# JeffreyXiang/ivid

Hardware: NVIDIA H100
Metric: 128x128 RGBD multiview samples/sec (higher is better)
Workload: dtype fp16 tensor-core operands, fp32 accumulate / residual stream / GroupNorm / softmax / sampler

## Files before the change

ivid_b200/csrc/elementwise.cuh:

```cuda
#pragma once
#include "common.cuh"

namespace ivid {

constexpr int kStatsPixPerBlock = 256;

__global__ void __launch_bounds__(256) gn_stats_kernel(const float* __restrict__ x, double* __restrict__ stats,
                                                       int HW, int C) {
  __shared__ float sred[256 * 8];
  const int n = blockIdx.y;
  const int c4 = C >> 2;
  const int cols = c4 < 256 ? c4 : 256;
  const int rows = 256 / cols;
  const int tx = threadIdx.x % cols;
  const int ty = threadIdx.x / cols;
  const int p0 = blockIdx.x * kStatsPixPerBlock;
  const int p1 = min(p0 + kStatsPixPerBlock, HW);
  const float* base = x + (static_cast<size_t>(n) * HW) * C;
  for (int cc = tx; cc < c4; cc += cols) {
    float s[4] = {0.f, 0.f, 0.f, 0.f}, q[4] = {0.f, 0.f, 0.f, 0.f};
    if (ty < rows) {
      for (int p = p0 + ty; p < p1; p += rows) {
        const float4 v = ldg_f4(base + static_cast<size_t>(p) * C + cc * 4);
        s[0] += v.x; s[1] += v.y; s[2] += v.z; s[3] += v.w;
        q[0] += v.x * v.x; q[1] += v.y * v.y; q[2] += v.z * v.z; q[3] += v.w * v.w;
      }
    }
    float* sm = sred;
    if (ty < rows) {
#pragma unroll
      for (int j = 0; j < 4; ++j) {
        sm[(ty * cols + tx) * 8 + j] = s[j];
        sm[(ty * cols + tx) * 8 + 4 + j] = q[j];
      }
    }
    __syncthreads();
    if (ty == 0) {
      double ds[4], dq[4];
#pragma unroll
      for (int j = 0; j < 4; ++j) { ds[j] = 0.0; dq[j] = 0.0; }
      for (int r = 0; r < rows; ++r) {
#pragma unroll
        for (int j = 0; j < 4; ++j) {
          ds[j] += static_cast<double>(sm[(r * cols + tx) * 8 + j]);
          dq[j] += static_cast<double>(sm[(r * cols + tx) * 8 + 4 + j]);
        }
      }
      double* o = stats + (static_cast<size_t>(n) * C + cc * 4) * 2;
#pragma unroll
      for (int j = 0; j < 4; ++j) {
        atomicAdd(o + 2 * j, ds[j]);
        atomicAdd(o + 2 * j + 1, dq[j]);
      }
    }
    __syncthreads();
  }
}

struct GnApplyParams {
  const float* x0; const float* x1;
  const __half* x0h; const __half* x1h;
  int C0, C1;
  int N, H, W;
  int mode;
  int silu;
  const double* stats0; const double* stats1;
  int groups; double inv_count; float eps;
  const float* gamma; const float* beta;
  const float* film; int film_ld, film_off;
  int film_add;
  int pix_per_block;
  __half* out_act;
  __half* out_lo;
  __half* out_raw16;
  float* out_raw32;
  uint8_t* out_act8;
};

template <bool kF8> struct Act8 { using T = uint4; };
template <> struct Act8<true> { using T = uint2; };
template <bool kF8>
__device__ __forceinline__ typename Act8<kF8>::T pack_act8(const float (&a)[8]) {
  if constexpr (kF8) {
    uint2 pk;
    pk.x = pack_e4m3x2(a[0], a[1]) | (static_cast<uint32_t>(pack_e4m3x2(a[2], a[3])) << 16);
    pk.y = pack_e4m3x2(a[4], a[5]) | (static_cast<uint32_t>(pack_e4m3x2(a[6], a[7])) << 16);
    return pk;
  } else {
    uint4 pk;
    pk.x = pack_h2(a[0], a[1]); pk.y = pack_h2(a[2], a[3]);
    pk.z = pack_h2(a[4], a[5]); pk.w = pack_h2(a[6], a[7]);
    return pk;
  }
}
template <bool kF8>
__device__ __forceinline__ void store_act8(const GnApplyParams& p, size_t o, const typename Act8<kF8>::T& v) {
  if constexpr (kF8) *reinterpret_cast<uint2*>(p.out_act8 + o) = v;
  else *reinterpret_cast<uint4*>(p.out_act + o) = v;
}

__device__ __forceinline__ void load8(const GnApplyParams& p, int n, int h, int w, int c, float (&v)[8]) {
  if (p.x0h != nullptr) {
    const __half* hs; int hc, hl;
    if (c < p.C0) { hs = p.x0h; hc = c; hl = p.C0; } else { hs = p.x1h; hc = c - p.C0; hl = p.C1; }
    const uint4 u = __ldg(reinterpret_cast<const uint4*>(hs + ((static_cast<size_t>(n) * p.H + h) * p.W + w) * hl + hc));
    const __half2* h2 = reinterpret_cast<const __half2*>(&u);
#pragma unroll
    for (int j = 0; j < 4; ++j) { const float2 f = __half22float2(h2[j]); v[2 * j] = f.x; v[2 * j + 1] = f.y; }
    return;
  }
  const float* src;
  int cc, ld;
  if (c < p.C0) { src = p.x0; cc = c; ld = p.C0; } else { src = p.x1; cc = c - p.C0; ld = p.C1; }
  const float* q = src + ((static_cast<size_t>(n) * p.H + h) * p.W + w) * ld + cc;
  const float4 a = ldg_f4(q), b = ldg_f4(q + 4);
  v[0] = a.x; v[1] = a.y; v[2] = a.z; v[3] = a.w; v[4] = b.x; v[5] = b.y; v[6] = b.z; v[7] = b.w;
}

__device__ __forceinline__ void gn_block_pos(const GnApplyParams&, int& n, int& bx) {
  n = static_cast<int>(blockIdx.y);
  bx = static_cast<int>(blockIdx.x);
}

__device__ __forceinline__ void gn_prologue(const GnApplyParams& p, float* s_ab, float* s_mean, float* s_rstd) {
  const int C = p.C0 + p.C1;
  int n, bx_unused;
  gn_block_pos(p, n, bx_unused);
  const int cpg = C / p.groups;
  if ((cpg & (cpg - 1)) == 0 && cpg <= 32 && C % 32 == 0 && C <= 4 * 256 && blockDim.x == 256) {
    constexpr int PF = 4;
    double2 st[PF];
    float pg[PF], pb[PF], psc[PF], psh[PF];
#pragma unroll
    for (int i = 0; i < PF; ++i) {
      const int c = threadIdx.x + i * 256;
      if (c < C) {
        const double* sp = (c < p.C0) ? p.stats0 + (static_cast<size_t>(n) * p.C0 + c) * 2
                                      : p.stats1 + (static_cast<size_t>(n) * p.C1 + (c - p.C0)) * 2;
        st[i] = *reinterpret_cast<const double2*>(sp);
        pg[i] = p.gamma[c];
        pb[i] = p.beta[c];
        if (p.film != nullptr) {
          psc[i] = p.film[static_cast<size_t>(n) * p.film_ld + p.film_off + c];
          psh[i] = p.film_add ? 0.f : p.film[static_cast<size_t>(n) * p.film_ld + p.film_off + C + c];
          if (p.film_add) {
            const double e = static_cast<double>(psc[i]), hw = 1.0 / p.inv_count;
            const double S = st[i].x;
            st[i].x = S + hw * e;
            st[i].y = st[i].y + 2.0 * e * S + hw * e * e;
          }
        }
      }
    }
    const double cnt_inv = p.inv_count / cpg;
#pragma unroll
    for (int i = 0; i < PF; ++i) {
      const int c = threadIdx.x + i * 256;
      if (c < C) {
        double sm = st[i].x, q = st[i].y;
        for (int off = 1; off < cpg; off <<= 1) {
          sm += __shfl_xor_sync(0xffffffffu, sm, off);
          q += __shfl_xor_sync(0xffffffffu, q, off);
        }
        const double mean = sm * cnt_inv;
        double var = q * cnt_inv - mean * mean;
        if (var < 0.0) var = 0.0;
        const float rstd = static_cast<float>(1.0 / sqrt(var + static_cast<double>(p.eps)));
        const float a0 = rstd * pg[i];
        const float b0 = pb[i] - static_cast<float>(mean) * a0;
        float av = a0, bv = b0;
        if (p.film != nullptr && p.film_add) {
          bv = fmaf(psc[i], a0, b0);
        } else if (p.film != nullptr) {
          const float sc = 1.0f + psc[i];
          av = a0 * sc;
          bv = b0 * sc + psh[i];
        }
        s_ab[(c & 7) * (C >> 3) + (c >> 3)] = av;
        s_ab[C + (c & 7) * (C >> 3) + (c >> 3)] = bv;
      }
    }
    __syncthreads();
    return;
  }
  for (int g = threadIdx.x; g < p.groups; g += blockDim.x) {
    double s = 0.0, q = 0.0;
    for (int c = g * cpg; c < (g + 1) * cpg; ++c) {
      const double* st = (c < p.C0) ? p.stats0 + (static_cast<size_t>(n) * p.C0 + c) * 2
                                    : p.stats1 + (static_cast<size_t>(n) * p.C1 + (c - p.C0)) * 2;
      double sc = st[0], qc = st[1];
      if (p.film != nullptr && p.film_add) {
        const double e = static_cast<double>(p.film[static_cast<size_t>(n) * p.film_ld + p.film_off + c]), hw = 1.0 / p.inv_count;
        qc = qc + 2.0 * e * sc + hw * e * e;
        sc = sc + hw * e;
      }
      s += sc;
      q += qc;
    }
    const double cnt_inv = p.inv_count / cpg;
    const double mean = s * cnt_inv;
    double var = q * cnt_inv - mean * mean;
    if (var < 0.0) var = 0.0;
    s_mean[g] = static_cast<float>(mean);
    s_rstd[g] = static_cast<float>(1.0 / sqrt(var + static_cast<double>(p.eps)));
  }
  __syncthreads();
  for (int c = threadIdx.x; c < C; c += blockDim.x) {
    const int g = c / cpg;
    const float a0 = s_rstd[g] * p.gamma[c];
    const float b0 = p.beta[c] - s_mean[g] * a0;
    float a = a0, b = b0;
    if (p.film != nullptr && p.film_add) {
      b = fmaf(p.film[static_cast<size_t>(n) * p.film_ld + p.film_off + c], a0, b0);
    } else if (p.film != nullptr) {
      const float sc = 1.0f + p.film[static_cast<size_t>(n) * p.film_ld + p.film_off + c];
      const float sh = p.film[static_cast<size_t>(n) * p.film_ld + p.film_off + C + c];
      a = a0 * sc;
      b = b0 * sc + sh;
    }
    s_ab[(c & 7) * (C >> 3) + (c >> 3)] = a;
    s_ab[C + (c & 7) * (C >> 3) + (c >> 3)] = b;
  }
  __syncthreads();

}

template <bool kF8 = false>
__global__ void __launch_bounds__(256, 3) gn_apply_kernel(const GnApplyParams p) {
  extern __shared__ float s_ab[];
  __shared__ float s_mean[64], s_rstd[64];
  gn_prologue(p, s_ab, s_mean, s_rstd);
  const int C = p.C0 + p.C1;
  int n, bx;
  gn_block_pos(p, n, bx);
  const int c8 = C >> 3;
  const int Ho = p.mode == 1 ? p.H * 2 : (p.mode == 2 ? p.H / 2 : p.H);
  const int Wo = p.mode == 1 ? p.W * 2 : (p.mode == 2 ? p.W / 2 : p.W);
  const int pix0 = bx * p.pix_per_block;
  if (p.mode == 1) {
    const int npix_s = min(p.pix_per_block, p.H * p.W - pix0);
    const int items_s = npix_s * c8;
    constexpr int U = 4;
    auto emit = [&](int it, const float (&raw)[8]) {
      const int cg = it % c8;
      const int pix = pix0 + it / c8;
      const int hs = pix / p.W, ws = pix - hs * p.W;
      float act[8];
#pragma unroll
      for (int j = 0; j < 8; ++j) {
        float y = fmaf(raw[j], s_ab[j * c8 + cg], s_ab[C + j * c8 + cg]);
        if (p.silu) y = silu_f(y);
        act[j] = y;
      }
      const auto pk = pack_act8<kF8>(act);
      const float4 r0 = make_float4(raw[0], raw[1], raw[2], raw[3]), r1 = make_float4(raw[4], raw[5], raw[6], raw[7]);
#pragma unroll
      for (int dy = 0; dy < 2; ++dy)
#pragma unroll
        for (int dx = 0; dx < 2; ++dx) {
          const size_t o = ((static_cast<size_t>(n) * Ho + 2 * hs + dy) * Wo + 2 * ws + dx) * C + cg * 8;
          store_act8<kF8>(p, o, pk);
          if (p.out_raw32 != nullptr) { stg_f4(p.out_raw32 + o, r0); stg_f4(p.out_raw32 + o + 4, r1); }
        }
    };
    int it0 = threadIdx.x;
    for (; it0 + (U - 1) * 256 < items_s; it0 += U * 256) {
      float raw[U][8];
#pragma unroll
      for (int u = 0; u < U; ++u) {
        const int it = it0 + u * 256;
        const int pix = pix0 + it / c8;
        load8(p, n, pix / p.W, pix % p.W, (it % c8) * 8, raw[u]);
      }
#pragma unroll
      for (int u = 0; u < U; ++u) emit(it0 + u * 256, raw[u]);
    }
    for (int it = it0; it < items_s; it += 256) {
      float raw[8];
      const int pix = pix0 + it / c8;
      load8(p, n, pix / p.W, pix % p.W, (it % c8) * 8, raw);
      emit(it, raw);
    }
    return;
  }
  const int npix = min(p.pix_per_block, Ho * Wo - pix0);
  const int items = npix * c8;
  int it0 = threadIdx.x;
  if (p.mode == 0) {
    constexpr int U = 4;
    for (; it0 + (U - 1) * 256 < items; it0 += U * 256) {
      float raw[U][8];
#pragma unroll
      for (int u = 0; u < U; ++u) {
        const int it = it0 + u * 256;
        const int pix = pix0 + it / c8;
        load8(p, n, pix / Wo, pix % Wo, (it % c8) * 8, raw[u]);
      }
#pragma unroll
      for (int u = 0; u < U; ++u) {
        const int it = it0 + u * 256;
        const int cg = it % c8;
        const int pix = pix0 + it / c8;
        const size_t o = (static_cast<size_t>(n) * Ho * Wo + pix) * C + cg * 8;
        float act[8];
#pragma unroll
        for (int j = 0; j < 8; ++j) {
          float y = fmaf(raw[u][j], s_ab[j * c8 + cg], s_ab[C + j * c8 + cg]);
          if (p.silu) y = silu_f(y);
          act[j] = y;
        }
        store_act8<kF8>(p, o, pack_act8<kF8>(act));
        if (p.out_raw16 != nullptr) {
          uint4 pr;
          pr.x = pack_h2(raw[u][0], raw[u][1]); pr.y = pack_h2(raw[u][2], raw[u][3]);
          pr.z = pack_h2(raw[u][4], raw[u][5]); pr.w = pack_h2(raw[u][6], raw[u][7]);
          *reinterpret_cast<uint4*>(p.out_raw16 + o) = pr;
        }
        if (p.out_raw32 != nullptr) {
          stg_f4(p.out_raw32 + o, make_float4(raw[u][0], raw[u][1], raw[u][2], raw[u][3]));
          stg_f4(p.out_raw32 + o + 4, make_float4(raw[u][4], raw[u][5], raw[u][6], raw[u][7]));
        }
      }
    }
  }
  for (int it = it0; it < items; it += blockDim.x) {
    const int cg = it % c8;
    const int pix = pix0 + it / c8;
    const int wo = pix % Wo, ho = pix / Wo;
    const int c = cg * 8;
    float A[8], B[8];
#pragma unroll
    for (int j = 0; j < 8; ++j) { A[j] = s_ab[j * c8 + cg]; B[j] = s_ab[C + j * c8 + cg]; }
    float act[8], raw[8];
    if (p.mode == 2) {
#pragma unroll
      for (int j = 0; j < 8; ++j) { act[j] = 0.f; raw[j] = 0.f; }
#pragma unroll
      for (int dy = 0; dy < 2; ++dy)
#pragma unroll
        for (int dx = 0; dx < 2; ++dx) {
          float v[8];
          load8(p, n, ho * 2 + dy, wo * 2 + dx, c, v);
#pragma unroll
          for (int j = 0; j < 8; ++j) {
            float y = fmaf(v[j], A[j], B[j]);
            if (p.silu) y = silu_f(y);
            act[j] += y;
            raw[j] += v[j];
          }
        }
#pragma unroll
      for (int j = 0; j < 8; ++j) { act[j] *= 0.25f; raw[j] *= 0.25f; }
    } else {
      const int hi = p.mode == 1 ? (ho >> 1) : ho;
      const int wi = p.mode == 1 ? (wo >> 1) : wo;
      load8(p, n, hi, wi, c, raw);
#pragma unroll
      for (int j = 0; j < 8; ++j) {
        float y = fmaf(raw[j], A[j], B[j]);
        if (p.silu) y = silu_f(y);
        act[j] = y;
      }
    }
    const size_t o = ((static_cast<size_t>(n) * Ho + ho) * Wo + wo) * C + c;
    store_act8<kF8>(p, o, pack_act8<kF8>(act));
    if (p.out_raw16 != nullptr) {
      uint4 pr;
      pr.x = pack_h2(raw[0], raw[1]); pr.y = pack_h2(raw[2], raw[3]);
      pr.z = pack_h2(raw[4], raw[5]); pr.w = pack_h2(raw[6], raw[7]);
      *reinterpret_cast<uint4*>(p.out_raw16 + o) = pr;
    }
    if (p.out_raw32 != nullptr) {
      stg_f4(p.out_raw32 + o, make_float4(raw[0], raw[1], raw[2], raw[3]));
      stg_f4(p.out_raw32 + o + 4, make_float4(raw[4], raw[5], raw[6], raw[7]));
    }
  }
}

__global__ void __launch_bounds__(256) im2col_s2_h16_kernel(const __half* __restrict__ x, __half* __restrict__ col, int N, int H, int W, int C) {
  const int Ho = H / 2, Wo = W / 2, c8 = C >> 3;
  const size_t total = static_cast<size_t>(N) * Ho * Wo * 9 * c8;
  for (size_t i = blockIdx.x * static_cast<size_t>(blockDim.x) + threadIdx.x; i < total; i += static_cast<size_t>(gridDim.x) * blockDim.x) {
    const int cg = static_cast<int>(i % c8);
    const int tap = static_cast<int>((i / c8) % 9);
    const size_t pix = i / (static_cast<size_t>(c8) * 9);
    const int xo = static_cast<int>(pix % Wo), yo = static_cast<int>((pix / Wo) % Ho);
    const int n = static_cast<int>(pix / (static_cast<size_t>(Wo) * Ho));
    const int yi = 2 * yo + tap / 3 - 1, xi = 2 * xo + tap % 3 - 1;
    uint4 v = make_uint4(0u, 0u, 0u, 0u);
    if (yi >= 0 && yi < H && xi >= 0 && xi < W)
      v = __ldg(reinterpret_cast<const uint4*>(x + ((static_cast<size_t>(n) * H + yi) * W + xi) * C + cg * 8));
    *reinterpret_cast<uint4*>(col + (pix * 9 + tap) * C + cg * 8) = v;
  }
}

__global__ void __launch_bounds__(256) upsample2x_h16_kernel(const __half* __restrict__ x, __half* __restrict__ out, int N, int H, int W, int C) {
  const int Ho = H * 2, Wo = W * 2, c8 = C >> 3;
  const size_t total = static_cast<size_t>(N) * Ho * Wo * c8;
  for (size_t i = blockIdx.x * static_cast<size_t>(blockDim.x) + threadIdx.x; i < total; i += static_cast<size_t>(gridDim.x) * blockDim.x) {
    const int cg = static_cast<int>(i % c8);
    const size_t pix = i / c8;
    const int xo = static_cast<int>(pix % Wo), yo = static_cast<int>((pix / Wo) % Ho);
    const int n = static_cast<int>(pix / (static_cast<size_t>(Wo) * Ho));
    *reinterpret_cast<uint4*>(out + pix * C + cg * 8) =
        __ldg(reinterpret_cast<const uint4*>(x + ((static_cast<size_t>(n) * H + (yo >> 1)) * W + (xo >> 1)) * C + cg * 8));
  }
}

__global__ void __launch_bounds__(256) resample_f32_kernel(const float* __restrict__ x, float* __restrict__ out, __half* __restrict__ out16,
                                                            int N, int H, int W, int C, int mode) {
  const int Ho = mode == 1 ? H * 2 : H / 2, Wo = mode == 1 ? W * 2 : W / 2, c4 = C >> 2;
  const size_t total = static_cast<size_t>(N) * Ho * Wo * c4;
  for (size_t i = blockIdx.x * static_cast<size_t>(blockDim.x) + threadIdx.x; i < total; i += static_cast<size_t>(gridDim.x) * blockDim.x) {
    const int cg = static_cast<int>(i % c4);
    const size_t pix = i / c4;
    const int xo = static_cast<int>(pix % Wo), yo = static_cast<int>((pix / Wo) % Ho);
    const int n = static_cast<int>(pix / (static_cast<size_t>(Wo) * Ho));
    float4 v;
    if (mode == 1) {
      v = ldg_f4(x + ((static_cast<size_t>(n) * H + (yo >> 1)) * W + (xo >> 1)) * C + cg * 4);
    } else {
      const float* b = x + ((static_cast<size_t>(n) * H + 2 * yo) * W + 2 * xo) * C + cg * 4;
      const float4 a0 = ldg_f4(b), a1 = ldg_f4(b + C), a2 = ldg_f4(b + static_cast<size_t>(W) * C), a3 = ldg_f4(b + static_cast<size_t>(W) * C + C);
      v = make_float4(((a0.x + a1.x) + (a2.x + a3.x)) * 0.25f, ((a0.y + a1.y) + (a2.y + a3.y)) * 0.25f,
                      ((a0.z + a1.z) + (a2.z + a3.z)) * 0.25f, ((a0.w + a1.w) + (a2.w + a3.w)) * 0.25f);
    }
    stg_f4(out + pix * C + cg * 4, v);
    if (out16 != nullptr) {
      uint2 pk;
      pk.x = pack_h2(v.x, v.y); pk.y = pack_h2(v.z, v.w);
      *reinterpret_cast<uint2*>(out16 + pix * C + cg * 4) = pk;
    }
  }
}

template <bool kHoist, bool kLo = false, bool kF8 = false>
__global__ void __launch_bounds__(256, 3) gn_apply_h16_kernel(const GnApplyParams p) {
  extern __shared__ float s_ab[];
  __shared__ float s_mean[64], s_rstd[64];
  gn_prologue(p, s_ab, s_mean, s_rstd);
  const int C = p.C0 + p.C1, c8 = C >> 3, c80 = p.C0 >> 3;
  int n, bx;
  gn_block_pos(p, n, bx);
  const int HW = p.H * p.W;
  const int pix0 = bx * p.pix_per_block;
  const int npix = min(p.pix_per_block, HW - pix0);
  const int items = npix * c8;
  constexpr int U = 8;
  float A[8], B[8];
  if (kHoist) {
    const int cg = threadIdx.x % c8;
#pragma unroll
    for (int j = 0; j < 8; ++j) { A[j] = s_ab[j * c8 + cg]; B[j] = s_ab[C + j * c8 + cg]; }
  }
  auto apply8 = [&](const uint4& rawv, int cg, __half* dst) {
    const __half2* h2 = reinterpret_cast<const __half2*>(&rawv);
    uint32_t pk[4], pl[4];
    uint16_t p8[4];
#pragma unroll
    for (int j = 0; j < 4; ++j) {
      const float2 f = __half22float2(h2[j]);
      float y0, y1;
      if (kHoist) {
        y0 = fmaf(f.x, A[2 * j], B[2 * j]);
        y1 = fmaf(f.y, A[2 * j + 1], B[2 * j + 1]);
      } else {
        y0 = fmaf(f.x, s_ab[(2 * j) * c8 + cg], s_ab[C + (2 * j) * c8 + cg]);
        y1 = fmaf(f.y, s_ab[(2 * j + 1) * c8 + cg], s_ab[C + (2 * j + 1) * c8 + cg]);
      }
      if (p.silu) { y0 = silu_f(y0); y1 = silu_f(y1); }
      if (kF8) { p8[j] = pack_e4m3x2(y0, y1); continue; }
      pk[j] = pack_h2(y0, y1);
      if (kLo) {
        const float2 hi = __half22float2(*reinterpret_cast<const __half2*>(&pk[j]));
        pl[j] = pack_h2(y0 - hi.x, y1 - hi.y);
      }
    }
    if (kF8) {
      *reinterpret_cast<uint2*>(p.out_act8 + (dst - p.out_act)) =
          make_uint2(p8[0] | (static_cast<uint32_t>(p8[1]) << 16), p8[2] | (static_cast<uint32_t>(p8[3]) << 16));
      return;
    }
    *reinterpret_cast<uint4*>(dst) = make_uint4(pk[0], pk[1], pk[2], pk[3]);
    if (kLo) *reinterpret_cast<uint4*>(p.out_lo + (dst - p.out_act)) = make_uint4(pl[0], pl[1], pl[2], pl[3]);
  };
  if (kHoist) {
    const int cg = threadIdx.x % c8, pr = threadIdx.x / c8, ppt = 256 / c8;
    const size_t px0 = static_cast<size_t>(n) * HW + pix0 + pr;
    const __half* src;
    size_t sstep;
    if (cg < c80) { src = p.x0h + px0 * p.C0 + cg * 8; sstep = static_cast<size_t>(ppt) * p.C0; }
    else { src = p.x1h + px0 * p.C1 + (cg - c80) * 8; sstep = static_cast<size_t>(ppt) * p.C1; }
    __half* dst = p.out_act + px0 * C + cg * 8;
    const size_t dstep = static_cast<size_t>(ppt) * C;
    int left = pr < npix ? (npix - pr + ppt - 1) / ppt : 0;
    for (; left >= U; left -= U) {
      uint4 raw[U];
#pragma unroll
      for (int u = 0; u < U; ++u) raw[u] = __ldg(reinterpret_cast<const uint4*>(src + u * sstep));
#pragma unroll
      for (int u = 0; u < U; ++u) apply8(raw[u], cg, dst + u * dstep);
      src += U * sstep;
      dst += U * dstep;
    }
    for (; left > 0; --left) {
      apply8(__ldg(reinterpret_cast<const uint4*>(src)), cg, dst);
      src += sstep;
      dst += dstep;
    }
    return;
  }
  auto src_of = [&](int it) {
    const int cg = it % c8;
    const size_t px = static_cast<size_t>(n) * HW + pix0 + it / c8;
    return cg < c80 ? p.x0h + px * p.C0 + cg * 8 : p.x1h + px * p.C1 + (cg - c80) * 8;
  };
  auto finish = [&](int it, const uint4& rawv) {
    apply8(rawv, it % c8, p.out_act + (static_cast<size_t>(n) * HW + pix0 + it / c8) * C + (it % c8) * 8);
  };
  int it0 = threadIdx.x;
  for (; it0 + (U - 1) * 256 < items; it0 += U * 256) {
    uint4 raw[U];
#pragma unroll
    for (int u = 0; u < U; ++u) raw[u] = __ldg(reinterpret_cast<const uint4*>(src_of(it0 + u * 256)));
#pragma unroll
    for (int u = 0; u < U; ++u) finish(it0 + u * 256, raw[u]);
  }
  for (int it = it0; it < items; it += 256) finish(it, __ldg(reinterpret_cast<const uint4*>(src_of(it))));
}

__global__ void __launch_bounds__(256) pack_input_kernel(const float* __restrict__ x, __half* __restrict__ out, int N,
                                                         int Nx, int Cin, int HW) {
  __shared__ float s_ch[256][17];
  const size_t total = static_cast<size_t>(N) * HW;
  for (size_t base = blockIdx.x * static_cast<size_t>(blockDim.x); base < total; base += static_cast<size_t>(gridDim.x) * blockDim.x) {
    const size_t idx = base + threadIdx.x;
    if (idx < total) {
      const int n = static_cast<int>(idx / HW);
      const int p = static_cast<int>(idx % HW);
      const float* src = x + (static_cast<size_t>(n % Nx) * Cin) * HW + p;
#pragma unroll
      for (int c = 0; c < 16; ++c) s_ch[threadIdx.x][c] = c < Cin ? __ldg(src + static_cast<size_t>(c) * HW) : 0.f;
    }
    __syncthreads();
    const int live = static_cast<int>(min(static_cast<size_t>(256), total - base));
    for (int it = threadIdx.x; it < live * 8; it += 256) {
      const int px = it >> 3, g = it & 7;
      uint32_t w[4];
#pragma unroll
      for (int k = 0; k < 4; ++k) {
        __half e[2];
#pragma unroll
        for (int q = 0; q < 2; ++q) {
          const int oc = g * 8 + 2 * k + q;
          const int seg = oc / Cin;
          e[q] = seg < 3 ? split_term(s_ch[px][oc - seg * Cin], seg) : __float2half_rn(0.f);
        }
        const __half2 h2 = __halves2half2(e[0], e[1]);
        w[k] = *reinterpret_cast<const uint32_t*>(&h2);
      }
      *reinterpret_cast<uint4*>(out + (base + px) * 64 + g * 8) = make_uint4(w[0], w[1], w[2], w[3]);
    }
    __syncthreads();
  }
}

__global__ void __launch_bounds__(256) eps_gather_kernel(const float* __restrict__ Y, const float* __restrict__ bias,
                                                         float* __restrict__ eps, int N, int H, int W, int Co, int ldy) {
  const size_t total = static_cast<size_t>(N) * H * W;
  for (size_t idx = blockIdx.x * static_cast<size_t>(blockDim.x) + threadIdx.x; idx < total;
       idx += static_cast<size_t>(gridDim.x) * blockDim.x) {
    const int w = static_cast<int>(idx % W);
    const int h = static_cast<int>((idx / W) % H);
    const int n = static_cast<int>(idx / (static_cast<size_t>(W) * H));
    float acc[8];
#pragma unroll
    for (int c = 0; c < 8; ++c) acc[c] = 0.f;
#pragma unroll
    for (int tap = 0; tap < 9; ++tap) {
      const int hh = h + tap / 3 - 1, ww = w + tap % 3 - 1;
      if (hh < 0 || hh >= H || ww < 0 || ww >= W) continue;
      const float* src = Y + ((static_cast<size_t>(n) * H + hh) * W + ww) * ldy + tap * Co;
      if (Co == 4) {
        const float4 v = ldg_f4(src);
        acc[0] += v.x; acc[1] += v.y; acc[2] += v.z; acc[3] += v.w;
      } else {
#pragma unroll
        for (int c = 0; c < 8; ++c) if (c < Co) acc[c] += __ldg(src + c);
      }
    }
#pragma unroll
    for (int c = 0; c < 8; ++c)
      if (c < Co) eps[((static_cast<size_t>(n) * Co + c) * H + h) * W + w] = acc[c] + __ldg(bias + c);
  }
}

}
```

ivid_b200/csrc/ops.cu:

```cuda
#include "ops.h"

#include <algorithm>
#include <cmath>
#include <mutex>

#include "attention.cuh"
#include "attention_hd.cuh"
#include "conv_gemm.cuh"
#include "elementwise.cuh"
#include "embed.cuh"

namespace ivid {

struct ConvLaunch {
  ConvMaps8 maps;
  ConvGemmParams p;
  int BN;
  bool a8;
  bool slab;
  int grid;
};

int conv_pad_cout(int cout) {
  if (cout >= 64) return ((cout + 63) / 64) * 64;
// ... 147 lines not shown
    M.b = Ktot > 0 ? make_weight_map(d.weight, d.cout_pad, Ktot, l->BN) : M.b8;
  } else {
    M.b = make_weight_map(d.weight, d.cout_pad, Ktot, l->BN);
  }
  int f32_ch = 0, f16_ch = 0;
  epilogue_box_channels(l->BN, l->slab, &f32_ch, &f16_ch);
  const auto f32 = CU_TENSOR_MAP_DATA_TYPE_FLOAT32;
  M.r = M.o = M.o16 = M.a[0];
  if (d.residual != nullptr) {
    const int up = p.res_up ? 1 : 0;
    M.r = make_act_map(d.residual, d.N, d.H >> up, d.W >> up, d.cout, p.TW >> up, p.TH >> up, p.TN, f32, d.ldr, f32_ch);
  }
  if (d.out_mode == 0) M.o = make_act_map(d.out, d.N, d.H, d.W, d.cout, p.TW, p.TH, p.TN, f32, d.ldc, f32_ch);
  const void* o16 = d.out_mode == 1 ? d.out : d.out_mode == 0 ? d.out16 : nullptr;
  if (o16 != nullptr) M.o16 = make_act_map(o16, d.N, d.H, d.W, d.cout, p.TW, p.TH, p.TN, CU_TENSOR_MAP_DATA_TYPE_FLOAT16, d.ldc, f16_ch);
  l->grid = p.tiles_w * p.tiles_h * p.tiles_n * p.n_blocks;
  return l;
}
void conv_launch_destroy(ConvLaunch* l) { delete l; }
int conv_launch_bn(const ConvLaunch* l) { return l->BN; }
bool conv_launch_a8(const ConvLaunch* l) { return l->a8; }

template <int BN, bool A8, bool SLAB>
static void run_conv(const ConvLaunch* l, cudaStream_t s) {
  using Cfg = ConvGemmCfg<BN, SLAB>;
  static std::once_flag once;
  std::call_once(once, [] {
    IVID_CHECK_CUDA(cudaFuncSetAttribute(conv_gemm_kernel<BN, A8, SLAB>, cudaFuncAttributeMaxDynamicSharedMemorySize, Cfg::SMEM_BYTES));
  });
  if constexpr (A8) conv_gemm_kernel<BN, true, SLAB><<<l->grid, Cfg::THREADS, Cfg::SMEM_BYTES, s>>>(l->maps, l->p);
  else conv_gemm_kernel<BN, false, SLAB><<<l->grid, Cfg::THREADS, Cfg::SMEM_BYTES, s>>>(static_cast<const ConvMaps&>(l->maps), l->p);
  IVID_CHECK_CUDA(cudaGetLastError());
}
template <bool A8, bool SLAB>
static void run_conv_bn(const ConvLaunch* l, cudaStream_t s) {
  switch (l->BN) {
    case 128: run_conv<128, A8, SLAB>(l, s); break;
    case 64: run_conv<64, A8, SLAB>(l, s); break;
    default: run_conv<16, A8, SLAB>(l, s); break;
  }
}
void conv_launch_run_out(const ConvLaunch* l, void* out, cudaStream_t s) {
  IVID_REQUIRE(l->p.out_mode == 2, "internal: only an NCHW conv output is patched at run time (NHWC outputs are in tensor maps)");
  ConvLaunch tmp = *l;
  tmp.p.out = out;
  conv_launch_run(&tmp, s);
}
void conv_launch_run(const ConvLaunch* l, cudaStream_t s) {
  if (l->a8) {
    if (l->slab) run_conv_bn<true, true>(l, s);
    else run_conv_bn<true, false>(l, s);
  } else {
    if (l->slab) run_conv_bn<false, true>(l, s);
    else run_conv_bn<false, false>(l, s);
  }
}

struct AttnLaunch {
  CUtensorMap mapQ, mapKV;
  AttnParams p;
  AttnHdParams hp;
  int head_ch = 64;
  int nv = 0;
  bool qres = false;
  int smem = 0;
  int grid;
};

AttnLaunch* attn_launch_create(const void* qkv, int N, int T, int C, int head_ch, void* out) {
  if (head_ch <= 0 || head_ch % 64 != 0)
    throw Error(kErrNotImplemented, "attention: head width " + std::to_string(head_ch) + " is not a multiple of 64");
  IVID_REQUIRE(C % head_ch == 0, "attention: channels must be a multiple of the head width " + std::to_string(head_ch));
  IVID_REQUIRE(T >= 1, "attention: sequence length must be positive");
  auto* l = new AttnLaunch();
  l->head_ch = head_ch;
  l->p.N = N; l->p.T = T; l->p.C = C; l->p.heads = C / 64;
  l->p.q_tiles = (T + 127) / 128;
  l->p.out = reinterpret_cast<__half*>(out);
  const uint64_t dims[3] = {static_cast<uint64_t>(3 * C), static_cast<uint64_t>(T), static_cast<uint64_t>(N)};
  const uint64_t str[2] = {static_cast<uint64_t>(3 * C) * 2, static_cast<uint64_t>(T) * 3 * C * 2};
  const uint32_t boxq[3] = {64, 128, 1};
  const uint32_t boxkv[3] = {64, AttnCfg::KV, 1};
  l->mapQ = make_tensor_map(CU_TENSOR_MAP_DATA_TYPE_FLOAT16, 3, const_cast<void*>(qkv), dims, str, boxq,
                            CU_TENSOR_MAP_SWIZZLE_128B);
  l->mapKV = make_tensor_map(CU_TENSOR_MAP_DATA_TYPE_FLOAT16, 3, const_cast<void*>(qkv), dims, str, boxkv,
                             CU_TENSOR_MAP_SWIZZLE_128B);
  l->grid = N * l->p.heads * l->p.q_tiles;
  if (head_ch == 64) return l;
  using Cfg = AttnHdCfg;
  const int k = head_ch / 64;
  const int slices = (k + 3) / 4;
  l->nv = (k + slices - 1) / slices;
  l->qres = k <= Cfg::RESIDENT_Q_MAX_CHUNKS;
  AttnHdParams& hp = l->hp;
  hp.N = N; hp.T = T; hp.C = C; hp.d = head_ch; hp.heads = C / head_ch; hp.chunks = k;
  hp.q_tiles = l->p.q_tiles;
  hp.slices = (k + l->nv - 1) / l->nv;
  hp.scale_log2 = static_cast<float>(1.4426950408889634 / std::sqrt(static_cast<double>(head_ch)));
  hp.out = l->p.out;
  const int q_bytes = l->qres ? k * Cfg::QCHUNK_BYTES : 0;
  const int fixed = q_bytes + 1024  + 1024 ;
  const int budget = l->nv == 2 ? Cfg::MAX_SMEM_2CTA : Cfg::MAX_SMEM;
  hp.stages = std::min(Cfg::MAX_STAGES, (budget - fixed) / Cfg::stage_bytes(l->qres));
  IVID_REQUIRE(hp.stages >= 4, "attention: shared-memory ring too shallow");
  l->smem = fixed + hp.stages * Cfg::stage_bytes(l->qres);
  l->grid = N * hp.heads * hp.q_tiles * hp.slices;
  return l;
}
void attn_launch_destroy(AttnLaunch* l) { delete l; }

template <int NV, bool QRES>
static void run_attn_hd(const AttnLaunch* l, cudaStream_t s) {
  static std::once_flag once;
  std::call_once(once, [] {
    IVID_CHECK_CUDA(cudaFuncSetAttribute(attention_hd_kernel<NV, QRES>, cudaFuncAttributeMaxDynamicSharedMemorySize, AttnHdCfg::MAX_SMEM));
  });
  attention_hd_kernel<NV, QRES><<<l->grid, AttnHdCfg::THREADS, l->smem, s>>>(l->mapQ, l->mapKV, l->hp);
  IVID_CHECK_CUDA(cudaGetLastError());
}

void attn_launch_run(const AttnLaunch* l, cudaStream_t s) {
  if (l->head_ch != 64) {
    switch (l->nv * 2 + (l->qres ? 1 : 0)) {
      case 5: run_attn_hd<2, true>(l, s); break;
      case 7: run_attn_hd<3, true>(l, s); break;
      case 9: run_attn_hd<4, true>(l, s); break;
      case 6: run_attn_hd<3, false>(l, s); break;
      case 8: run_attn_hd<4, false>(l, s); break;
      default: throw Error(kErrState, "internal: attention slice width " + std::to_string(l->nv));
    }
    return;
  }
  static std::once_flag once;
  std::call_once(once, [] {
    IVID_CHECK_CUDA(cudaFuncSetAttribute(attention_kernel, cudaFuncAttributeMaxDynamicSharedMemorySize, AttnCfg::SMEM_BYTES));
  });
  attention_kernel<<<l->grid, AttnCfg::THREADS, AttnCfg::SMEM_BYTES, s>>>(l->mapQ, l->mapKV, l->p);
  IVID_CHECK_CUDA(cudaGetLastError());
}

static int ew_grid(size_t work_items, int block) {
  const size_t blocks = (work_items + block - 1) / block;
  const size_t cap = static_cast<size_t>(sm_count()) * 16;
  return static_cast<int>(std::max<size_t>(1, std::min(blocks, cap)));
}

void launch_gn_stats(const float* x, double* stats, int N, int HW, int C, cudaStream_t s) {
  IVID_REQUIRE(C % 4 == 0, "gn_stats: C % 4");
  dim3 grid((HW + kStatsPixPerBlock - 1) / kStatsPixPerBlock, N);
  gn_stats_kernel<<<grid, 256, 0, s>>>(x, stats, HW, C);
  IVID_CHECK_CUDA(cudaGetLastError());
}

void launch_gn_apply(const GnApplyDesc& d, cudaStream_t s) {
  IVID_REQUIRE(d.C0 % 8 == 0 && d.C1 % 8 == 0, "gn_apply: channel counts must be multiples of 8");
  const int C = d.C0 + d.C1;
  IVID_REQUIRE(d.groups >= 1 && d.groups <= 64 && C % d.groups == 0, "group norm: groups must divide channels (<= 64 groups)");
  IVID_REQUIRE(d.stats0 != nullptr && d.gamma != nullptr && d.beta != nullptr, "gn_apply: statistics / affine parameters missing");
  GnApplyParams p;
  p.x0 = static_cast<const float*>(d.x0); p.x1 = static_cast<const float*>(d.x1); p.C0 = d.C0; p.C1 = d.C1; p.N = d.N; p.H = d.H; p.W = d.W; p.mode = d.mode;
  p.x0h = d.x0_half ? reinterpret_cast<const __half*>(d.x0) : nullptr;
  p.x1h = d.x0_half ? reinterpret_cast<const __half*>(d.x1) : nullptr;
  p.silu = d.silu ? 1 : 0;
  p.stats0 = d.stats0; p.stats1 = d.stats1; p.groups = d.groups; p.inv_count = 1.0 / (static_cast<double>(d.H) * d.W);
  p.eps = d.eps; p.gamma = d.gamma; p.beta = d.beta; p.film = d.film; p.film_ld = d.film_ld; p.film_off = d.film_off;
  p.film_add = d.film_add ? 1 : 0;
  p.out_act = reinterpret_cast<__half*>(d.out_act); p.out_raw16 = reinterpret_cast<__half*>(d.out_raw16);
  p.out_act8 = d.out_e4m3 ? reinterpret_cast<uint8_t*>(d.out_act) : nullptr;
  p.out_raw32 = d.out_raw32;
  p.out_lo = reinterpret_cast<__half*>(d.out_lo);
  IVID_REQUIRE(d.out_lo == nullptr || (d.mode == 0 && d.x0_half && d.out_raw16 == nullptr && d.out_raw32 == nullptr),
               "gn_apply: the split (hi/lo) output exists on the same-resolution fp16-source path only");
  IVID_REQUIRE(!d.out_e4m3 || (d.out_lo == nullptr && C % 16 == 0), "gn_apply: an e4m3 output needs C % 16 == 0 and no split output");
  const int Ho = d.mode == 1 ? d.H * 2 : (d.mode == 2 ? d.H / 2 : d.H);
  const int Wo = d.mode == 1 ? d.W * 2 : (d.mode == 2 ? d.W / 2 : d.W);
  {
    const int blocks_per_n = std::max(1, (sm_count() * 3) / std::max(d.N, 1));
    const int by_wave = (Ho * Wo + blocks_per_n - 1) / blocks_per_n;
    const int small = std::max(1, 1024 / (C / 8));
    p.pix_per_block = std::max(1, std::min(Ho * Wo, std::max(by_wave, small)));
  }
  int pix_space = Ho * Wo;
  if (d.mode == 1) {
    pix_space = d.H * d.W;
    p.pix_per_block = std::max(1, (p.pix_per_block + 3) / 4);
  }
  dim3 grid((pix_space + p.pix_per_block - 1) / p.pix_per_block, d.N);
  const size_t smem = static_cast<size_t>(C) * 8;
  if (p.mode == 0 && p.x0h != nullptr && p.out_raw16 == nullptr && p.out_raw32 == nullptr) {
    const bool hoist = 256 % (C / 8) == 0;
    if (p.out_lo != nullptr) {
      if (hoist) gn_apply_h16_kernel<true, true><<<grid, 256, smem, s>>>(p);
      else gn_apply_h16_kernel<false, true><<<grid, 256, smem, s>>>(p);
    } else if (d.out_e4m3) {
      if (hoist) gn_apply_h16_kernel<true, false, true><<<grid, 256, smem, s>>>(p);
      else gn_apply_h16_kernel<false, false, true><<<grid, 256, smem, s>>>(p);
    } else if (hoist) gn_apply_h16_kernel<true><<<grid, 256, smem, s>>>(p);
    else gn_apply_h16_kernel<false><<<grid, 256, smem, s>>>(p);
  } else if (d.out_e4m3) {
    gn_apply_kernel<true><<<grid, 256, smem, s>>>(p);
  } else {
    gn_apply_kernel<><<<grid, 256, smem, s>>>(p);
  }
  IVID_CHECK_CUDA(cudaGetLastError());
}
void launch_im2col_s2(const void* x16, void* col, int N, int H, int W, int C, cudaStream_t s) {
  IVID_REQUIRE(C % 8 == 0 && H % 2 == 0 && W % 2 == 0, "im2col_s2: C % 8, even spatial size");
  const size_t items = static_cast<size_t>(N) * (H / 2) * (W / 2) * 9 * (C / 8);
  im2col_s2_h16_kernel<<<ew_grid(items, 256), 256, 0, s>>>(reinterpret_cast<const __half*>(x16), reinterpret_cast<__half*>(col), N, H, W, C);
  IVID_CHECK_CUDA(cudaGetLastError());
}
void launch_upsample2x_h16(const void* x16, void* out, int N, int H, int W, int C, cudaStream_t s) {
  IVID_REQUIRE(C % 8 == 0, "upsample2x: C % 8");
  const size_t items = static_cast<size_t>(N) * H * W * 4 * (C / 8);
  upsample2x_h16_kernel<<<ew_grid(items, 256), 256, 0, s>>>(reinterpret_cast<const __half*>(x16), reinterpret_cast<__half*>(out), N, H, W, C);
  IVID_CHECK_CUDA(cudaGetLastError());
}
void launch_resample_f32(const float* x, float* out, void* out16, int N, int H, int W, int C, int mode, cudaStream_t s) {
  IVID_REQUIRE(C % 4 == 0 && (mode == 1 || (H % 2 == 0 && W % 2 == 0)), "resample_f32: C % 4, even spatial size for pooling");
  const size_t items = static_cast<size_t>(N) * (mode == 1 ? 4 * H * W : (H / 2) * (W / 2)) * (C / 4);
  resample_f32_kernel<<<ew_grid(items, 256), 256, 0, s>>>(x, out, reinterpret_cast<__half*>(out16), N, H, W, C, mode);
  IVID_CHECK_CUDA(cudaGetLastError());
}
void launch_pack_input(const float* x, void* out, int N, int Nx, int Cin, int HW, cudaStream_t s) {
  IVID_REQUIRE(Cin >= 1 && Cin <= 16, "pack_input: 1..16 input channels (two-term split inside 64 operand channels)");
  pack_input_kernel<<<ew_grid(static_cast<size_t>(N) * HW, 256), 256, 0, s>>>(x, reinterpret_cast<__half*>(out), N, Nx,
                                                                                 Cin, HW);
  IVID_CHECK_CUDA(cudaGetLastError());
}

void launch_eps_gather(const float* Y, const float* bias, float* eps, int N, int H, int W, int Co, int ldy, cudaStream_t s) {
  IVID_REQUIRE(Co >= 1 && Co <= 7 && 9 * Co <= ldy, "eps_gather: 9*Co tap columns must fit the row pitch");
  IVID_REQUIRE(Co != 4 || ldy % 4 == 0, "eps_gather: row pitch must keep float4 alignment");
  eps_gather_kernel<<<ew_grid(static_cast<size_t>(N) * H * W, 256), 256, 0, s>>>(Y, bias, eps, N, H, W, Co, ldy);
  IVID_CHECK_CUDA(cudaGetLastError());
}

void launch_posenc(const int64_t* t, int Nt, const float* freqs, int half, float* out, int N, cudaStream_t s) {
  posenc_kernel<<<N, 128, 0, s>>>(t, Nt, freqs, half, out, N);
  IVID_CHECK_CUDA(cudaGetLastError());
}

void launch_film_table(const float* emb, const float* Wp, const float* bias, float* x_t, float* out, int N, int K, int O, cudaStream_t s) {
  IVID_REQUIRE(K % 32 == 0 && O % 4 == 0, "film table: K % 32 == 0");
  static std::once_flag once;
  std::call_once(once, [] {
    IVID_CHECK_CUDA(cudaFuncSetAttribute(film_table_kernel, cudaFuncAttributeMaxDynamicSharedMemorySize, FilmCfg::SMEM_BYTES));
  });
  const int nblk = (N + 31) / 32;
  silu_transpose_kernel<<<std::min(256, (nblk * K * 32 + 255) / 256), 256, 0, s>>>(emb, x_t, N, K, 1);
  const int tiles = (O + FilmCfg::TO - 1) / FilmCfg::TO;
  dim3 grid(std::min(tiles, std::max(1, sm_count() / nblk)), nblk);
  film_table_kernel<<<grid, FilmCfg::THREADS, FilmCfg::SMEM_BYTES, s>>>(Wp, x_t, bias, out, N, K, O);
  IVID_CHECK_CUDA(cudaGetLastError());
}

void launch_linear(const float* in, const float* W, const float* bias, float* out, int N, int K, int O, int silu_in,
                   const float* label_emb, const int64_t* classes, int Ncls, cudaStream_t s) {
  if ((K == 256 || K == 512 || K == 1024) && O <= 8192) {
    dim3 grid((O + 7) / 8, (N + 31) / 32);
    const size_t smem = static_cast<size_t>(32) * K * 4;
    static std::once_flag once;
    std::call_once(once, [] {
      IVID_CHECK_CUDA(cudaFuncSetAttribute(linear_warp_kernel<2>, cudaFuncAttributeMaxDynamicSharedMemorySize, 32 * 256 * 4));
      IVID_CHECK_CUDA(cudaFuncSetAttribute(linear_warp_kernel<4>, cudaFuncAttributeMaxDynamicSharedMemorySize, 32 * 512 * 4));
      IVID_CHECK_CUDA(cudaFuncSetAttribute(linear_warp_kernel<8>, cudaFuncAttributeMaxDynamicSharedMemorySize, 32 * 1024 * 4));
    });
    auto go = [&](auto kern) { kern<<<grid, 256, smem, s>>>(in, W, bias, out, N, O, silu_in, label_emb, classes, Ncls); };
    if (K == 256) go(linear_warp_kernel<2>); else if (K == 512) go(linear_warp_kernel<4>); else go(linear_warp_kernel<8>);
    IVID_CHECK_CUDA(cudaGetLastError());
    return;
  }
  if (K % 32 == 0) {
    if (O >= 128 * 64) {
      dim3 grid((O + 127) / 128, (N + 31) / 32);
      linear_tiled_kernel<4><<<grid, 256, 0, s>>>(in, W, bias, out, N, K, O, silu_in, label_emb, classes, Ncls);
    } else {
      dim3 grid((O + 63) / 64, (N + 31) / 32);
      linear_tiled_kernel<2><<<grid, 256, 0, s>>>(in, W, bias, out, N, K, O, silu_in, label_emb, classes, Ncls);
    }
    IVID_CHECK_CUDA(cudaGetLastError());
    return;
  }
  dim3 grid((O + 63) / 64, (N + 31) / 32);
  linear_rows_kernel<<<grid, 256, 0, s>>>(in, W, bias, out, N, K, O, silu_in, label_emb, classes, Ncls);
  IVID_CHECK_CUDA(cudaGetLastError());
}

}
```

Measured before the change: 0.3518.

## Slice fp16 GroupNorm apply by channel chunks and prefetch loads before coefficients

```diff
diff --git a/ivid_b200/csrc/elementwise.cuh b/ivid_b200/csrc/elementwise.cuh
--- a/ivid_b200/csrc/elementwise.cuh
+++ b/ivid_b200/csrc/elementwise.cuh
@@ -70,6 +70,7 @@
   const float* film; int film_ld, film_off;
   int film_add;
   int pix_per_block;
+  int cb;
   __half* out_act;
   __half* out_lo;
   __half* out_raw16;
@@ -117,24 +118,19 @@
   v[0] = a.x; v[1] = a.y; v[2] = a.z; v[3] = a.w; v[4] = b.x; v[5] = b.y; v[6] = b.z; v[7] = b.w;
 }
 
-__device__ __forceinline__ void gn_block_pos(const GnApplyParams&, int& n, int& bx) {
-  n = static_cast<int>(blockIdx.y);
-  bx = static_cast<int>(blockIdx.x);
-}
-
-__device__ __forceinline__ void gn_prologue(const GnApplyParams& p, float* s_ab, float* s_mean, float* s_rstd) {
+template <int PF>
+__device__ __forceinline__ void gn_coeffs(const GnApplyParams& p, int n, int c_lo, int nc, float* s_ab, float* s_mean,
+                                          float* s_rstd) {
   const int C = p.C0 + p.C1;
-  int n, bx_unused;
-  gn_block_pos(p, n, bx_unused);
   const int cpg = C / p.groups;
+  const int c8 = nc >> 3;
   if ((cpg & (cpg - 1)) == 0 && cpg <= 32 && C % 32 == 0 && C <= 4 * 256 && blockDim.x == 256) {
-    constexpr int PF = 4;
     double2 st[PF];
     float pg[PF], pb[PF], psc[PF], psh[PF];
 #pragma unroll
     for (int i = 0; i < PF; ++i) {
-      const int c = threadIdx.x + i * 256;
-      if (c < C) {
+      const int c = c_lo + threadIdx.x + i * 256;
+      if (threadIdx.x + i * 256 < nc) {
         const double* sp = (c < p.C0) ? p.stats0 + (static_cast<size_t>(n) * p.C0 + c) * 2
                                       : p.stats1 + (static_cast<size_t>(n) * p.C1 + (c - p.C0)) * 2;
         st[i] = *reinterpret_cast<const double2*>(sp);
@@ -155,8 +151,8 @@
     const double cnt_inv = p.inv_count / cpg;
 #pragma unroll
     for (int i = 0; i < PF; ++i) {
-      const int c = threadIdx.x + i * 256;
-      if (c < C) {
+      const int l = threadIdx.x + i * 256;
+      if (l < nc) {
         double sm = st[i].x, q = st[i].y;
         for (int off = 1; off < cpg; off <<= 1) {
           sm += __shfl_xor_sync(0xffffffffu, sm, off);
@@ -176,16 +172,20 @@
           av = a0 * sc;
           bv = b0 * sc + psh[i];
         }
-        s_ab[(c & 7) * (C >> 3) + (c >> 3)] = av;
-        s_ab[C + (c & 7) * (C >> 3) + (c >> 3)] = bv;
+        s_ab[(l & 7) * c8 + (l >> 3)] = av;
+        s_ab[nc + (l & 7) * c8 + (l >> 3)] = bv;
       }
     }
     __syncthreads();
     return;
   }
-  for (int g = threadIdx.x; g < p.groups; g += blockDim.x) {
-    double s = 0.0, q = 0.0;
-    for (int c = g * cpg; c < (g + 1) * cpg; ++c) {
+  __shared__ double2 s_st[256];
+  const int g0 = c_lo / cpg, g1 = (c_lo + nc - 1) / cpg + 1;
+  const int g = g0 + static_cast<int>(threadIdx.x);
+  double s = 0.0, q = 0.0;
+  for (int base = g0 * cpg; base < g1 * cpg; base += 256) {
+    const int c = base + static_cast<int>(threadIdx.x);
+    if (c < g1 * cpg) {
       const double* st = (c < p.C0) ? p.stats0 + (static_cast<size_t>(n) * p.C0 + c) * 2
                                     : p.stats1 + (static_cast<size_t>(n) * p.C1 + (c - p.C0)) * 2;
       double sc = st[0], qc = st[1];
@@ -194,19 +194,31 @@
         qc = qc + 2.0 * e * sc + hw * e * e;
         sc = sc + hw * e;
       }
-      s += sc;
-      q += qc;
-    }
+      s_st[threadIdx.x] = make_double2(sc, qc);
+    }
+    __syncthreads();
+    if (g < g1) {
+      const int e0 = max(g * cpg, base), e1 = min((g + 1) * cpg, base + 256);
+#pragma unroll 1
+      for (int cc = e0; cc < e1; ++cc) {
+        s += s_st[cc - base].x;
+        q += s_st[cc - base].y;
+      }
+    }
+    __syncthreads();
+  }
+  if (g < g1) {
     const double cnt_inv = p.inv_count / cpg;
     const double mean = s * cnt_inv;
     double var = q * cnt_inv - mean * mean;
     if (var < 0.0) var = 0.0;
-    s_mean[g] = static_cast<float>(mean);
-    s_rstd[g] = static_cast<float>(1.0 / sqrt(var + static_cast<double>(p.eps)));
+    s_mean[g - g0] = static_cast<float>(mean);
+    s_rstd[g - g0] = static_cast<float>(1.0 / sqrt(var + static_cast<double>(p.eps)));
   }
   __syncthreads();
-  for (int c = threadIdx.x; c < C; c += blockDim.x) {
-    const int g = c / cpg;
+  for (int l = threadIdx.x; l < nc; l += blockDim.x) {
+    const int c = c_lo + l;
+    const int g = c / cpg - g0;
     const float a0 = s_rstd[g] * p.gamma[c];
     const float b0 = p.beta[c] - s_mean[g] * a0;
     float a = a0, b = b0;
@@ -218,11 +230,14 @@
       a = a0 * sc;
       b = b0 * sc + sh;
     }
-    s_ab[(c & 7) * (C >> 3) + (c >> 3)] = a;
-    s_ab[C + (c & 7) * (C >> 3) + (c >> 3)] = b;
+    s_ab[(l & 7) * c8 + (l >> 3)] = a;
+    s_ab[nc + (l & 7) * c8 + (l >> 3)] = b;
   }
   __syncthreads();
-
+}
+
+__device__ __forceinline__ void gn_prologue(const GnApplyParams& p, float* s_ab, float* s_mean, float* s_rstd) {
+  gn_coeffs<4>(p, static_cast<int>(blockIdx.y), 0, p.C0 + p.C1, s_ab, s_mean, s_rstd);
 }
 
 template <bool kF8 = false>
@@ -231,8 +246,7 @@
   __shared__ float s_mean[64], s_rstd[64];
   gn_prologue(p, s_ab, s_mean, s_rstd);
   const int C = p.C0 + p.C1;
-  int n, bx;
-  gn_block_pos(p, n, bx);
+  const int n = static_cast<int>(blockIdx.y), bx = static_cast<int>(blockIdx.x);
   const int c8 = C >> 3;
   const int Ho = p.mode == 1 ? p.H * 2 : (p.mode == 2 ? p.H / 2 : p.H);
   const int Wo = p.mode == 1 ? p.W * 2 : (p.mode == 2 ? p.W / 2 : p.W);
@@ -434,40 +448,49 @@
   }
 }
 
-template <bool kHoist, bool kLo = false, bool kF8 = false>
+template <bool kLo = false, bool kF8 = false>
 __global__ void __launch_bounds__(256, 3) gn_apply_h16_kernel(const GnApplyParams p) {
-  extern __shared__ float s_ab[];
+  __shared__ float s_ab[2 * 256];
   __shared__ float s_mean[64], s_rstd[64];
-  gn_prologue(p, s_ab, s_mean, s_rstd);
-  const int C = p.C0 + p.C1, c8 = C >> 3, c80 = p.C0 >> 3;
-  int n, bx;
-  gn_block_pos(p, n, bx);
+  const int n = p.N - 1 - static_cast<int>(blockIdx.z);
+  const int chunk = static_cast<int>(gridDim.x - 1 - blockIdx.x);
+  const int c8 = p.cb >> 3, c_lo = static_cast<int>(blockIdx.y) * p.cb;
+  const int C = p.C0 + p.C1, c80 = p.C0 >> 3;
   const int HW = p.H * p.W;
-  const int pix0 = bx * p.pix_per_block;
+  const int pix0 = chunk * p.pix_per_block;
   const int npix = min(p.pix_per_block, HW - pix0);
-  const int items = npix * c8;
   constexpr int U = 8;
+  const int cl = threadIdx.x & (c8 - 1), pr = threadIdx.x / c8, ppt = 256 / c8;
+  const int cg = (c_lo >> 3) + cl;
+  const size_t px0 = static_cast<size_t>(n) * HW + pix0 + pr;
+  const __half* src;
+  size_t sstep;
+  if (cg < c80) { src = p.x0h + px0 * p.C0 + cg * 8; sstep = static_cast<size_t>(ppt) * p.C0; }
+  else { src = p.x1h + px0 * p.C1 + (cg - c80) * 8; sstep = static_cast<size_t>(ppt) * p.C1; }
+  __half* dst = p.out_act + px0 * C + cg * 8;
+  const size_t dstep = static_cast<size_t>(ppt) * C;
+  int left = pr < npix ? (npix - pr + ppt - 1) / ppt : 0;
+  uint4 raw[U];
+  auto load_trip = [&](int k) {
+#pragma unroll
+    for (int u = 0; u < U; ++u)
+      if (u < k) raw[u] = __ldg(reinterpret_cast<const uint4*>(src + u * sstep));
+  };
+  const int k = kLo ? 0 : min(left, U);
+  load_trip(k);
+  gn_coeffs<1>(p, n, c_lo, p.cb, s_ab, s_mean, s_rstd);
   float A[8], B[8];
-  if (kHoist) {
-    const int cg = threadIdx.x % c8;
-#pragma unroll
-    for (int j = 0; j < 8; ++j) { A[j] = s_ab[j * c8 + cg]; B[j] = s_ab[C + j * c8 + cg]; }
-  }
-  auto apply8 = [&](const uint4& rawv, int cg, __half* dst) {
+#pragma unroll
+  for (int j = 0; j < 8; ++j) { A[j] = s_ab[j * c8 + cl]; B[j] = s_ab[p.cb + j * c8 + cl]; }
+  auto apply8 = [&](const uint4& rawv, __half* dst) {
     const __half2* h2 = reinterpret_cast<const __half2*>(&rawv);
     uint32_t pk[4], pl[4];
     uint16_t p8[4];
 #pragma unroll
     for (int j = 0; j < 4; ++j) {
       const float2 f = __half22float2(h2[j]);
-      float y0, y1;
-      if (kHoist) {
-        y0 = fmaf(f.x, A[2 * j], B[2 * j]);
-        y1 = fmaf(f.y, A[2 * j + 1], B[2 * j + 1]);
-      } else {
-        y0 = fmaf(f.x, s_ab[(2 * j) * c8 + cg], s_ab[C + (2 * j) * c8 + cg]);
-        y1 = fmaf(f.y, s_ab[(2 * j + 1) * c8 + cg], s_ab[C + (2 * j + 1) * c8 + cg]);
-      }
+      float y0 = fmaf(f.x, A[2 * j], B[2 * j]);
+      float y1 = fmaf(f.y, A[2 * j + 1], B[2 * j + 1]);
       if (p.silu) { y0 = silu_f(y0); y1 = silu_f(y1); }
       if (kF8) { p8[j] = pack_e4m3x2(y0, y1); continue; }
       pk[j] = pack_h2(y0, y1);
@@ -484,49 +507,22 @@
     *reinterpret_cast<uint4*>(dst) = make_uint4(pk[0], pk[1], pk[2], pk[3]);
     if (kLo) *reinterpret_cast<uint4*>(p.out_lo + (dst - p.out_act)) = make_uint4(pl[0], pl[1], pl[2], pl[3]);
   };
-  if (kHoist) {
-    const int cg = threadIdx.x % c8, pr = threadIdx.x / c8, ppt = 256 / c8;
-    const size_t px0 = static_cast<size_t>(n) * HW + pix0 + pr;
-    const __half* src;
-    size_t sstep;
-    if (cg < c80) { src = p.x0h + px0 * p.C0 + cg * 8; sstep = static_cast<size_t>(ppt) * p.C0; }
-    else { src = p.x1h + px0 * p.C1 + (cg - c80) * 8; sstep = static_cast<size_t>(ppt) * p.C1; }
-    __half* dst = p.out_act + px0 * C + cg * 8;
-    const size_t dstep = static_cast<size_t>(ppt) * C;
-    int left = pr < npix ? (npix - pr + ppt - 1) / ppt : 0;
-    for (; left >= U; left -= U) {
-      uint4 raw[U];
-#pragma unroll
-      for (int u = 0; u < U; ++u) raw[u] = __ldg(reinterpret_cast<const uint4*>(src + u * sstep));
-#pragma unroll
-      for (int u = 0; u < U; ++u) apply8(raw[u], cg, dst + u * dstep);
-      src += U * sstep;
-      dst += U * dstep;
-    }
-    for (; left > 0; --left) {
-      apply8(__ldg(reinterpret_cast<const uint4*>(src)), cg, dst);
-      src += sstep;
-      dst += dstep;
-    }
-    return;
-  }
-  auto src_of = [&](int it) {
-    const int cg = it % c8;
-    const size_t px = static_cast<size_t>(n) * HW + pix0 + it / c8;
-    return cg < c80 ? p.x0h + px * p.C0 + cg * 8 : p.x1h + px * p.C1 + (cg - c80) * 8;
+  auto apply_trip = [&](int k) {
+#pragma unroll
+    for (int u = 0; u < U; ++u)
+      if (u < k) apply8(raw[u], dst + u * dstep);
+    src += U * sstep;
+    dst += U * dstep;
   };
-  auto finish = [&](int it, const uint4& rawv) {
-    apply8(rawv, it % c8, p.out_act + (static_cast<size_t>(n) * HW + pix0 + it / c8) * C + (it % c8) * 8);
-  };
-  int it0 = threadIdx.x;
-  for (; it0 + (U - 1) * 256 < items; it0 += U * 256) {
-    uint4 raw[U];
-#pragma unroll
-    for (int u = 0; u < U; ++u) raw[u] = __ldg(reinterpret_cast<const uint4*>(src_of(it0 + u * 256)));
-#pragma unroll
-    for (int u = 0; u < U; ++u) finish(it0 + u * 256, raw[u]);
-  }
-  for (int it = it0; it < items; it += 256) finish(it, __ldg(reinterpret_cast<const uint4*>(src_of(it))));
+  if (k > 0) apply_trip(k);
+  for (left -= k; left >= U; left -= U) {
+    load_trip(U);
+    apply_trip(U);
+  }
+  if (left > 0) {
+    load_trip(left);
+    apply_trip(left);
+  }
 }
 
 __global__ void __launch_bounds__(256) pack_input_kernel(const float* __restrict__ x, __half* __restrict__ out, int N,
diff --git a/ivid_b200/csrc/ops.cu b/ivid_b200/csrc/ops.cu
--- a/ivid_b200/csrc/ops.cu
+++ b/ivid_b200/csrc/ops.cu
@@ -323,6 +323,26 @@
   IVID_CHECK_CUDA(cudaGetLastError());
 }
 
+static int gn_h16_slice(int C) {
+  int cb = 8;
+  while (cb < 256 && C % (2 * cb) == 0) cb *= 2;
+  return cb;
+}
+static int gn_h16_pixels(int N, int HW, int C, int cb) {
+  const int ppt = 256 / (cb / 8);
+  const long long rows = (HW + ppt - 1) / ppt;
+  const long long units = static_cast<long long>(N) * (C / cb);
+  const long long wave = static_cast<long long>(sm_count()) * 3;
+  int best = 1;
+  long long best_cost = -1;
+  for (int t = 1; t <= 16; ++t) {
+    const long long waves = (units * ((rows + t - 1) / t) + wave - 1) / wave;
+    const long long cost = waves * (t + 1);
+    if (best_cost < 0 || cost < best_cost) { best = t; best_cost = cost; }
+  }
+  return ppt * best;
+}
+
 void launch_gn_apply(const GnApplyDesc& d, cudaStream_t s) {
   IVID_REQUIRE(d.C0 % 8 == 0 && d.C1 % 8 == 0, "gn_apply: channel counts must be multiples of 8");
   const int C = d.C0 + d.C1;
@@ -343,6 +363,16 @@
   IVID_REQUIRE(d.out_lo == nullptr || (d.mode == 0 && d.x0_half && d.out_raw16 == nullptr && d.out_raw32 == nullptr),
                "gn_apply: the split (hi/lo) output exists on the same-resolution fp16-source path only");
   IVID_REQUIRE(!d.out_e4m3 || (d.out_lo == nullptr && C % 16 == 0), "gn_apply: an e4m3 output needs C % 16 == 0 and no split output");
+  if (p.mode == 0 && p.x0h != nullptr && p.out_raw16 == nullptr && p.out_raw32 == nullptr) {
+    p.cb = gn_h16_slice(C);
+    p.pix_per_block = gn_h16_pixels(d.N, d.H * d.W, C, p.cb);
+    const dim3 grid((d.H * d.W + p.pix_per_block - 1) / p.pix_per_block, C / p.cb, d.N);
+    if (p.out_lo != nullptr) gn_apply_h16_kernel<true><<<grid, 256, 0, s>>>(p);
+    else if (d.out_e4m3) gn_apply_h16_kernel<false, true><<<grid, 256, 0, s>>>(p);
+    else gn_apply_h16_kernel<><<<grid, 256, 0, s>>>(p);
+    IVID_CHECK_CUDA(cudaGetLastError());
+    return;
+  }
   const int Ho = d.mode == 1 ? d.H * 2 : (d.mode == 2 ? d.H / 2 : d.H);
   const int Wo = d.mode == 1 ? d.W * 2 : (d.mode == 2 ? d.W / 2 : d.W);
   {
@@ -358,17 +388,7 @@
   }
   dim3 grid((pix_space + p.pix_per_block - 1) / p.pix_per_block, d.N);
   const size_t smem = static_cast<size_t>(C) * 8;
-  if (p.mode == 0 && p.x0h != nullptr && p.out_raw16 == nullptr && p.out_raw32 == nullptr) {
-    const bool hoist = 256 % (C / 8) == 0;
-    if (p.out_lo != nullptr) {
-      if (hoist) gn_apply_h16_kernel<true, true><<<grid, 256, smem, s>>>(p);
-      else gn_apply_h16_kernel<false, true><<<grid, 256, smem, s>>>(p);
-    } else if (d.out_e4m3) {
-      if (hoist) gn_apply_h16_kernel<true, false, true><<<grid, 256, smem, s>>>(p);
-      else gn_apply_h16_kernel<false, false, true><<<grid, 256, smem, s>>>(p);
-    } else if (hoist) gn_apply_h16_kernel<true><<<grid, 256, smem, s>>>(p);
-    else gn_apply_h16_kernel<false><<<grid, 256, smem, s>>>(p);
-  } else if (d.out_e4m3) {
+  if (d.out_e4m3) {
     gn_apply_kernel<true><<<grid, 256, smem, s>>>(p);
   } else {
     gn_apply_kernel<><<<grid, 256, smem, s>>>(p);
```

Measured after the change: 0.3541, median of 6. No clear change (+0.7%).
